# V-DETR/V-DETR

Hardware: AMD Instinct MI355X
Metric: scenes/sec (train fwd+bwd) 40k-pt ScanNet (higher is better)
Workload: dtype f32

## Files before the change

### include/vdetr_hip.h

```cpp
#ifndef VDETR_HIP_H
#define VDETR_HIP_H

#include <stddef.h>
#include <stdint.h>

#ifdef __cplusplus
extern "C" {
#endif

#define VDETR_OK 0
#define VDETR_ERR_ARG 1
#define VDETR_ERR_LAUNCH 2
#define VDETR_ERR_WORKSPACE 3

typedef void* vdetr_stream_t;

int vdetr_abi_version(void);
const char* vdetr_last_error(void);
int vdetr_ab_switches(void);


size_t vdetr_fps_workspace_bytes(int b, int n);
int vdetr_furthest_point_sampling_f32(const float* xyz, int b, int n, int m, int32_t* idx,
                                      void* workspace, size_t workspace_bytes, vdetr_stream_t stream);
// ... 327 lines not shown
  float *save_mean, *save_invstd;
  const float* pre_bias;
  int64_t* counters[8];
  int32_t ncounters;
  int32_t stats_given;
} vdetr_bnact_desc;

typedef struct vdetr_bnact_grads {
  const float* dy;
  float* dx;
  float *d_gamma, *d_beta;
  const float *sum_dy_xhat, *sum_dy, *inv_count;
} vdetr_bnact_grads;

int vdetr_relu_dropout_fwd_f32(const float* x, float* y, long n, float dropout_p, uint64_t seed, uint64_t offset,
                               const uint64_t* rng_state, vdetr_stream_t stream);
int vdetr_relu_dropout_bwd_f32(const float* y, const float* dy, float* dx, long n, float dropout_p, vdetr_stream_t stream);
int vdetr_bn_act_fwd_f32(const vdetr_bnact_desc* d, vdetr_stream_t stream);
int vdetr_bn_stats_f32(const vdetr_bnact_desc* d, float* mean, float* m2, vdetr_stream_t stream);
int vdetr_bn_act_bwd_f32(const vdetr_bnact_desc* d, const vdetr_bnact_grads* g, vdetr_stream_t stream);
int vdetr_bn_act_bwd_batch_f32(const vdetr_bnact_desc* descs, const vdetr_bnact_grads* grads, int n, vdetr_stream_t stream);

typedef struct vdetr_pack_entry {
  const void* src;
  uint64_t dst_offset;
  uint64_t numel;
} vdetr_pack_entry;
int vdetr_colsum_f32(const float* x, float* out, int rows, int cols, long row_stride, vdetr_stream_t stream);
size_t vdetr_colsum_workspace_bytes(int n, int rows, int cols);
int vdetr_colsum_batched_f32(const float* x, float* out, int n, int rows, int cols, long row_stride, long item_stride,
                             void* workspace, size_t workspace_bytes, vdetr_stream_t stream);
int vdetr_colsum_ptrs_f32(const float* const* items, float* out, int n, int rows, int cols, long row_stride, void* workspace,
                          size_t workspace_bytes, vdetr_stream_t stream);
int vdetr_pack_chunk_floats(void);
int vdetr_pack_f32(const vdetr_pack_entry* entries, const uint32_t* block_entry, const uint32_t* block_chunk, int nblocks,
                   float* dst, vdetr_stream_t stream);
int vdetr_pack_sumsq_f32(const vdetr_pack_entry* entries, const uint32_t* block_entry, const uint32_t* block_chunk, int nblocks,
                         float* dst, float* sumsq, vdetr_stream_t stream);

int vdetr_cpb_tables_f32(const float* coords, const float* w1, const float* b1, const float* w2, int n, int P, int hidden, int H,
                         float* hid_out, float* tables, vdetr_stream_t stream);

typedef struct vdetr_adamw_desc {
  float* param;
  const float* grad;
  float* exp_avg;
  float* exp_avg_sq;
  int64_t n;
  float* step;
  uint32_t* ticket;
  const float* sumsq;
  int32_t nsumsq;
  float max_norm;
  float norm_eps;
  float* norm_out;
  double lr, beta1, beta2, eps, weight_decay;
} vdetr_adamw_desc;
int vdetr_adamw_clip_f32(const vdetr_adamw_desc* d, vdetr_stream_t stream);
int vdetr_sumsq_blocks(long n);
int vdetr_sumsq_f32(const float* g, long n, float* partial, int npartial, vdetr_stream_t stream);

int vdetr_morton_sort_max(void);
int vdetr_morton_order_f32(const float* xyz, int B, int n, int* codes, long long* order, vdetr_stream_t stream);
int vdetr_topk_order_f32(const float* values, int B, int n, int nq, long long* order, vdetr_stream_t stream);

#define VDETR_GT_CORNERS 0
// ... 217 lines not shown
```

### v-detr_amd/_lib.py

```python
import ctypes
import os

import torch

_HERE = os.path.dirname(os.path.abspath(__file__))
LIB_PATH = os.path.join(_HERE, "lib", "libvdetr_hip.so")

c_int, c_float, c_void_p, c_size_t = ctypes.c_int, ctypes.c_float, ctypes.c_void_p, ctypes.c_size_t

VDETR_ATTN_SHARED_KV, VDETR_ATTN_PER_HEAD = 0, 1
VDETR_MASK_NONE, VDETR_MASK_BOOL, VDETR_MASK_FLOAT = 0, 1, 2


class AttnDesc(ctypes.Structure):

    _fields_ = [
        ("kind", ctypes.c_int32), ("B", ctypes.c_int32), ("H", ctypes.c_int32), ("nQ", ctypes.c_int32),
        ("nK", ctypes.c_int32), ("scale", c_float),
        ("table", c_void_p), ("table_size", ctypes.c_int32), ("log_scale", c_float), ("inv_log_norm", c_float),
        ("vertices", c_void_p), ("xyz", c_void_p), ("cos_sin", c_void_p),
        ("mask", c_void_p), ("mask_kind", ctypes.c_int32),
        ("dropout_p", c_float), ("seed", ctypes.c_uint64), ("offset", ctypes.c_uint64),
        ("rng_state", c_void_p),
        ("k_row_stride", ctypes.c_int32), ("v_row_stride", ctypes.c_int32),
# ... 182 lines not shown

class LsaProblem(ctypes.Structure):

    _fields_ = [(n, c_void_p) for n in ("cost_t", "nactual", "inds", "mask")] + [
        (n, ctypes.c_int32) for n in ("B", "P", "G", "row_repeat")]


class LsaBatch(ctypes.Structure):

    _fields_ = [("nproblems", ctypes.c_int32), ("reserved", ctypes.c_int32), ("p", LsaProblem * VDETR_LSA_MAX_PROBLEMS)]


_LOSS_W = ("w_cls", "w_angle_cls", "w_angle_reg", "w_center", "w_size", "w_giou")
_LOSS_PTR = ("cls_logits", "center_reg", "size_reg", "pre_center", "pre_size", "corners", "angle_logits", "angle_res_norm",
             "gt", "nactual", "inds", "mask", "labels", "num_boxes", "losses", "card_ws", "d_cls_logits", "d_center_reg", "d_size_reg",
             "d_corners", "d_angle_logits", "d_angle_res_norm", "rotated", "ce_rows_matched")


class SetLossDesc(ctypes.Structure):

    _fields_ = ([(n, ctypes.c_int32) for n in ("B", "P", "G", "C", "A", "label_override")] + [("focal_alpha", c_float)] +
                [(n, c_float) for n in _LOSS_W] + [("cls_kind", ctypes.c_int32), ("w_no_object", c_float)] +
                [(n, c_void_p) for n in _LOSS_PTR])


VDETR_IOU_GIOU, VDETR_IOU_DIOU, VDETR_IOU_IOU = 0, 1, 2
IOU_KINDS = {"giou": VDETR_IOU_GIOU, "diou": VDETR_IOU_DIOU, "iou": VDETR_IOU_IOU}


class IouExt(ctypes.Structure):

    _fields_ = [("iou_kind", ctypes.c_int32), ("reserved", ctypes.c_int32)] + [
        (n, c_void_p) for n in ("center", "size", "angle", "d_center", "d_size", "d_angle")]


class SpBnDesc(ctypes.Structure):

    _fields_ = ([(n, ctypes.c_int32) for n in ("N", "C", "act", "training")] + [("eps", c_float), ("momentum", c_float)] +
                [(n, c_void_p) for n in ("x", "gamma", "beta", "residual", "running_mean", "running_var", "num_batches_tracked",
                                         "y", "save_mean", "save_invstd", "workspace")])


_SIGNATURES = {
    "vdetr_abi_version": (c_int, []),
    "vdetr_ab_switches": (c_int, []),
    "vdetr_last_error": (ctypes.c_char_p, []),
    "vdetr_fps_workspace_bytes": (c_size_t, [c_int, c_int]),
    "vdetr_furthest_point_sampling_f32": (c_int, [c_void_p, c_int, c_int, c_int, c_void_p, c_void_p, c_size_t, c_void_p]),
    "vdetr_fps_varlen_workspace_bytes": (c_size_t, [c_void_p, c_int]),
    "vdetr_furthest_point_sampling_varlen_f32": (c_int, [c_void_p, c_void_p, c_int, c_int, c_void_p, c_void_p, c_size_t, c_void_p]),
    "vdetr_pos_embed_fourier_f32": (c_int, [c_void_p, c_int, c_int, c_void_p, c_void_p, c_void_p, c_int, c_int, c_void_p, c_void_p]),
    "vdetr_pos_embed_sine_f32": (c_int, [c_void_p, c_int, c_int, c_void_p, c_void_p, c_int, c_float, c_float, c_void_p, c_void_p]),
    "vdetr_gather_rows_f32": (c_int, [c_void_p, c_void_p, c_void_p, c_int, c_int, c_int, c_void_p]),
    "vdetr_gather_rows_grad_f32": (c_int, [c_void_p, c_void_p, c_void_p, c_int, c_int, c_int, c_void_p]),
    "vdetr_gather_points_f32": (c_int, [c_void_p, c_void_p, c_void_p, c_int, c_int, c_int, c_int, c_void_p]),
    "vdetr_gather_points_grad_f32": (c_int, [c_void_p, c_void_p, c_void_p, c_int, c_int, c_int, c_int, c_void_p]),
    "vdetr_gather_points_grad_set_f32": (c_int, [c_void_p, c_void_p, c_void_p, c_int, c_int, c_int, c_int, c_void_p]),
    "vdetr_group_points_grad_set_f32": (c_int, [c_void_p, c_void_p, c_void_p, c_int, c_int, c_int, c_int, c_int, c_void_p]),
    "vdetr_ball_query_f32": (c_int, [c_void_p, c_void_p, c_void_p, c_int, c_int, c_int, c_float, c_int, c_void_p]),
    "vdetr_group_points_f32": (c_int, [c_void_p, c_void_p, c_void_p, c_int, c_int, c_int, c_int, c_int, c_void_p]),
    "vdetr_group_points_grad_f32": (c_int, [c_void_p, c_void_p, c_void_p, c_int, c_int, c_int, c_int, c_int, c_void_p]),
    "vdetr_three_nn_f32": (c_int, [c_void_p, c_void_p, c_void_p, c_void_p, c_int, c_int, c_int, c_void_p]),
    "vdetr_three_interpolate_f32": (c_int, [c_void_p, c_void_p, c_void_p, c_void_p, c_int, c_int, c_int, c_int, c_void_p]),
    "vdetr_three_interpolate_grad_f32": (c_int, [c_void_p, c_void_p, c_void_p, c_void_p, c_int, c_int, c_int, c_int, c_void_p]),
    "vdetr_attn_fwd_workspace_bytes": (c_size_t, [ctypes.POINTER(AttnDesc)]),
    "vdetr_attn_kv_image_bytes": (c_size_t, [c_int, c_int]),
# ... 8 lines not shown
    "vdetr_attn_bwd_scores_f32": (c_int, [ctypes.POINTER(AttnDesc), c_void_p, c_void_p, c_void_p, c_void_p, c_void_p, c_void_p, c_void_p, c_void_p, c_size_t, c_void_p]),
    "vdetr_attn_bwd_kv_workspace_bytes": (c_size_t, [ctypes.POINTER(AttnDesc)]),
    "vdetr_attn_bwd_kv_f32": (c_int, [ctypes.POINTER(AttnDesc)] + [c_void_p] * 10 + [c_size_t, c_void_p]),
    "vdetr_attn_bwd_kv_delta_f32": (c_int, [ctypes.POINTER(AttnDesc)] + [c_void_p] * 11 + [c_size_t, c_void_p]),
    "vdetr_attn_bwd_dq_f32": (c_int, [ctypes.POINTER(AttnDesc), c_void_p, c_void_p, c_void_p, c_void_p]),
    "vdetr_attn_bwd_table_f32": (c_int, [ctypes.POINTER(AttnDesc), c_void_p, c_void_p, c_void_p, c_size_t, c_void_p]),
    "vdetr_attn_bwd_table_kernel_names": (c_int, [ctypes.POINTER(AttnDesc), ctypes.POINTER(ctypes.c_char_p), ctypes.POINTER(ctypes.c_char_p)]),
    "vdetr_attn_delta_f32": (c_int, [ctypes.POINTER(AttnDesc), c_void_p, c_void_p, c_void_p, c_void_p, c_void_p]),
    "vdetr_attn_dropout_mask_u8": (c_int, [ctypes.POINTER(AttnDesc), c_void_p, c_void_p]),
    "vdetr_rpe_bias_f32": (c_int, [ctypes.POINTER(AttnDesc), c_void_p, c_void_p]),
    "vdetr_box_decode_fwd_f32": (c_int, [ctypes.POINTER(BoxDecodeDesc), c_void_p]),
    "vdetr_box_decode_bwd_f32": (c_int, [ctypes.POINTER(BoxDecodeDesc), ctypes.POINTER(BoxDecodeGrads), c_void_p]),
    "vdetr_box_decode_bwd_batch_f32": (c_int, [ctypes.POINTER(BoxDecodeDesc), ctypes.POINTER(BoxDecodeGrads), c_int, c_void_p]),
    "vdetr_add_ln_fwd_f32": (c_int, [ctypes.POINTER(AddLnDesc), c_void_p]),
    "vdetr_add_ln_bwd_workspace_bytes": (c_size_t, [ctypes.POINTER(AddLnDesc)]),
    "vdetr_add_ln_bwd_f32": (c_int, [ctypes.POINTER(AddLnDesc), ctypes.POINTER(AddLnGrads), c_void_p]),
    "vdetr_add_ln_param_reduce_batch_f32": (c_int, [ctypes.POINTER(AddLnReduce), c_int, c_void_p]),
    "vdetr_relu_dropout_fwd_f32": (c_int, [c_void_p, c_void_p, ctypes.c_long, c_float, ctypes.c_uint64, ctypes.c_uint64, c_void_p,
                                           c_void_p]),
    "vdetr_relu_dropout_bwd_f32": (c_int, [c_void_p, c_void_p, c_void_p, ctypes.c_long, c_float, c_void_p]),
    "vdetr_bn_act_fwd_f32": (c_int, [ctypes.POINTER(BnActDesc), c_void_p]),
    "vdetr_bn_stats_f32": (c_int, [ctypes.POINTER(BnActDesc), c_void_p, c_void_p, c_void_p]),
    "vdetr_heads_workspace_bytes": (c_size_t, [c_int, c_int, c_int]),
    "vdetr_heads_fwd_f32": (c_int, [ctypes.POINTER(HeadsDesc), c_void_p]),
    "vdetr_pos_mlp_fwd_f32": (c_int, [ctypes.POINTER(PosMlpDesc), c_void_p]),
    "vdetr_heads_infer_f32": (c_int, [ctypes.POINTER(HeadsInferDesc), c_void_p]),
    "vdetr_pos_mlp_infer_f32": (c_int, [ctypes.POINTER(PosMlpDesc), c_void_p]),
    "vdetr_bn_act_bwd_f32": (c_int, [ctypes.POINTER(BnActDesc), ctypes.POINTER(BnActGrads), c_void_p]),
    "vdetr_bn_act_bwd_batch_f32": (c_int, [ctypes.POINTER(BnActDesc), ctypes.POINTER(BnActGrads), c_int, c_void_p]),
    "vdetr_colsum_f32": (c_int, [c_void_p, c_void_p, c_int, c_int, ctypes.c_long, c_void_p]),
    "vdetr_colsum_workspace_bytes": (c_size_t, [c_int, c_int, c_int]),
    "vdetr_colsum_batched_f32": (c_int, [c_void_p, c_void_p, c_int, c_int, c_int, ctypes.c_long, ctypes.c_long, c_void_p, c_size_t, c_void_p]),
    "vdetr_colsum_ptrs_f32": (c_int, [c_void_p, c_void_p, c_int, c_int, c_int, ctypes.c_long, c_void_p, c_size_t, c_void_p]),
    "vdetr_nms3d_workspace_bytes": (c_size_t, [c_int, c_int]),
    "vdetr_nms3d_f32": (c_int, [c_void_p, c_void_p, c_void_p, c_void_p, c_void_p, c_int, c_int, ctypes.c_double, c_int, c_void_p,
                        c_void_p, c_size_t, c_void_p]),
    "vdetr_nms3d_rot_workspace_bytes": (c_size_t, [c_int, c_int]),
    "vdetr_nms3d_rot_f32": (c_int, [c_void_p, c_void_p, c_void_p, c_void_p, c_void_p, c_int, c_int, ctypes.c_double, c_int, c_void_p,
                            c_void_p, c_size_t, c_void_p]),
    "vdetr_box_point_count_f32": (c_int, [c_void_p, c_void_p, c_int, c_int, c_int, c_void_p, c_void_p]),
    "vdetr_box3d_iou_max_f64": (c_int, [c_void_p, c_void_p, c_void_p, c_int, c_void_p, c_void_p, c_void_p, c_void_p, c_void_p,
                                c_void_p]),
    "vdetr_box3d_iou_pairs_f64": (c_int, [c_void_p, c_int, c_void_p, c_int, c_void_p, c_void_p]),
    "vdetr_morton_sort_max": (c_int, []),
    "vdetr_morton_order_f32": (c_int, [c_void_p, c_int, c_int, c_void_p, c_void_p, c_void_p]),
    "vdetr_pack_chunk_floats": (c_int, []),
    "vdetr_pack_f32": (c_int, [c_void_p, c_void_p, c_void_p, c_int, c_void_p, c_void_p]),
    "vdetr_pack_sumsq_f32": (c_int, [c_void_p, c_void_p, c_void_p, c_int, c_void_p, c_void_p, c_void_p]),
    "vdetr_adamw_clip_f32": (c_int, [ctypes.POINTER(AdamWDesc), c_void_p]),
    "vdetr_cpb_tables_f32": (c_int, [c_void_p] * 4 + [c_int] * 4 + [c_void_p] * 3),
    "vdetr_sumsq_blocks": (c_int, [ctypes.c_long]),
    "vdetr_sumsq_f32": (c_int, [c_void_p, ctypes.c_long, c_void_p, c_int, c_void_p]),
    "vdetr_gt_prepare_f32": (c_int, [c_void_p, c_int, c_int, c_int, c_void_p, c_void_p, c_void_p, c_void_p, c_void_p]),
    "vdetr_match_cost_f32": (c_int, [ctypes.POINTER(MatchDesc), c_void_p]),
    "vdetr_match_cost_batch_f32": (c_int, [ctypes.POINTER(MatchDesc), c_int, c_void_p]),
    "vdetr_lsa_f64": (c_int, [ctypes.POINTER(LsaBatch), c_void_p, c_void_p]),
    "vdetr_point_labels_f32": (c_int, [c_void_p, c_void_p, c_void_p, c_int, c_int, c_int, c_int, c_void_p, c_void_p, c_void_p]),
    "vdetr_set_loss_f32": (c_int, [ctypes.POINTER(SetLossDesc), c_void_p]),
    "vdetr_set_loss_batch_f32": (c_int, [ctypes.POINTER(SetLossDesc), c_int, c_void_p]),
    "vdetr_match_cost_ext_batch_f32": (c_int, [ctypes.POINTER(MatchDesc), ctypes.POINTER(IouExt), c_int, c_void_p]),
    "vdetr_set_loss_ext_batch_f32": (c_int, [ctypes.POINTER(SetLossDesc), ctypes.POINTER(IouExt), c_int, c_void_p]),
    "vdetr_sp_kernel_map_i32": (c_int, [c_void_p, c_int, c_void_p, c_int, c_void_p, c_int, c_void_p, c_void_p]),
    "vdetr_sp_inverse_map_i32": (c_int, [c_void_p, c_int, c_int, c_int, c_void_p, c_void_p]),
    "vdetr_sp_gather_cols_f32": (c_int, [c_void_p, c_void_p, c_int, c_int, c_int, c_void_p, c_void_p]),
    "vdetr_sp_gather_sum_f32": (c_int, [c_void_p, c_void_p, c_int, c_int, c_int, c_int, c_void_p, c_void_p]),
    "vdetr_sp_pairs_gemm_f32": (c_int, [c_void_p, c_void_p, c_void_p, c_void_p, c_int, c_int, c_int, c_int, c_void_p, c_void_p]),
# ... 60 lines not shown

def stream_ptr():
    return c_void_p(torch.cuda.current_stream().cuda_stream)


def ptr(t):
    return c_void_p(t.data_ptr()) if t is not None else c_void_p(0)


def require_gpu(t, name):
    if not t.is_cuda:
        raise RuntimeError(f"{name}: CPU not supported (tensor is on {t.device})")


def require_contiguous(t, name):
    if not t.is_contiguous():
        raise RuntimeError(f"{name} must be a contiguous tensor")


def require_float(t, name):
    if t.dtype != torch.float32:
        raise RuntimeError(f"{name} must be a float tensor")


def require_int(t, name):
    if t.dtype != torch.int32:
        raise RuntimeError(f"{name} must be an int tensor")


def workspace(nbytes, device):
    return torch.empty(max(int(nbytes), 1), dtype=torch.uint8, device=device)


_rocblas = {"lib": None, "handles": {}}
ROCBLAS_OP_N, ROCBLAS_OP_T = 111, 112


def rocblas():
    if _rocblas["lib"] is None:
        path = os.path.join(os.path.dirname(torch.__file__), "lib", "librocblas.so")
        rb = ctypes.CDLL(path if os.path.exists(path) else "librocblas.so")
        rb.rocblas_create_handle.argtypes = [ctypes.POINTER(c_void_p)]
        rb.rocblas_set_stream.argtypes = [c_void_p, c_void_p]
        rb.rocblas_sgemm_batched.argtypes = [c_void_p, c_int, c_int, c_int, c_int, c_int, c_void_p, c_void_p, c_int, c_void_p, c_int,
                                             c_void_p, c_void_p, c_int, c_int]
        _rocblas["lib"] = rb
    return _rocblas["lib"]


def sgemm_batched_ptrs(op_a, op_b, m, n, k, a_ptrs, lda, b_ptrs, ldb, c_ptrs, ldc, batch, device, alpha=1.0, beta=0.0):
    rb = rocblas()
    key = device.index if device.index is not None else torch.cuda.current_device()
    h = _rocblas["handles"].get(key)
    if h is None:
        if torch.cuda.is_current_stream_capturing():
            raise RuntimeError("rocBLAS handle: create it before a stream capture (run one step eagerly first)")
        h = c_void_p()
        with torch.cuda.device(key):
            if rb.rocblas_create_handle(ctypes.byref(h)) != 0:
                raise RuntimeError("rocblas_create_handle failed")
        _rocblas["handles"][key] = h
    if rb.rocblas_set_stream(h, c_void_p(torch.cuda.current_stream(device).cuda_stream)) != 0:
        raise RuntimeError("rocblas_set_stream failed")
    al, be = c_float(alpha), c_float(beta)
    addr = lambda p: c_void_p(p.data_ptr() if torch.is_tensor(p) else int(p))
    rc = rb.rocblas_sgemm_batched(h, op_a, op_b, m, n, k, ctypes.byref(al), addr(a_ptrs), lda, addr(b_ptrs), ldb, ctypes.byref(be),
                                  addr(c_ptrs), ldc, batch)
    if rc != 0:
        raise RuntimeError(f"rocblas_sgemm_batched failed (status {rc})")


_ptr_tables = {}


def upload_ptrs(ptrs, device):
    n = len(ptrs)
    key = device.index if device.index is not None else torch.cuda.current_device()
    T = _ptr_tables.get(key)
    if T is None:
        if torch.cuda.is_current_stream_capturing():
            raise RuntimeError("pointer tables: allocate before a stream capture (run one step eagerly first)")
        T = _ptr_tables[key] = {"ring": [torch.empty(1024, dtype=torch.int64).pin_memory() for _ in range(4)], "events": [None] * 4, "tick": 0,
                                "spare": [torch.empty(1024, dtype=torch.int64).pin_memory() for _ in range(48)], "kept": []}
    if n > 1024:
        raise RuntimeError(f"pointer table of {n} entries (max 1024)")
    dev = torch.empty(n, dtype=torch.int64, device=device)
    if torch.cuda.is_current_stream_capturing():
        if not T["spare"]:
            raise RuntimeError("pointer tables: more than 48 captured uploads in this process")
        host = T["spare"].pop()
        T["kept"].append(host)
        host[:n] = torch.tensor(ptrs, dtype=torch.int64)
        dev.copy_(host[:n], non_blocking=True)
        return dev
    slot = T["tick"] % 4
    T["tick"] += 1
    if T["events"][slot] is not None:
        T["events"][slot].synchronize()
    host = T["ring"][slot]
    host[:n] = torch.tensor(ptrs, dtype=torch.int64)
    dev.copy_(host[:n], non_blocking=True)
    ev = torch.cuda.Event()
    ev.record(torch.cuda.current_stream(device))
    T["events"][slot] = ev
    return dev
```

### v-detr_amd/helpers.py

```python
import copy
import os
from functools import partial

import torch
import torch.nn as nn


def colsum_batched(x3d):
    import ctypes
    from . import _lib as L
    assert x3d.dim() == 3 and x3d.stride(2) == 1
    n, rows, cols = x3d.shape
    lib = L.lib()
    need = lib.vdetr_colsum_workspace_bytes(n, rows, cols)
    ws = torch.empty(need, dtype=torch.uint8, device=x3d.device) if need else None
    out = torch.empty((n, cols), dtype=x3d.dtype, device=x3d.device)
    L.check(lib.vdetr_colsum_batched_f32(L.ptr(x3d), L.ptr(out), n, rows, cols, ctypes.c_long(x3d.stride(1)), ctypes.c_long(x3d.stride(0)),
                                         L.ptr(ws), need, L.stream_ptr()), "colsum_batched")
    return out


PTR_BATCH = os.environ.get("VDETR_PTR_BATCH", "1") != "0"


def _ptr_batchable(group):
    if not PTR_BATCH or len(group) > 256 or len(group) < 8:
        return False
    if torch.distributed.is_available() and torch.distributed.is_initialized() and torch.distributed.get_world_size() > 1:
        return False
    g0, x0 = group[0][2], group[0][3]
    if g0.shape[0] > 1024:
        return False
    if not (g0.is_cuda and g0.dtype == torch.float32 and x0.dtype == torch.float32 and g0.shape[1] % 4 == 0):
        return False
    for it in group:
        g, x = it[2], it[3]
        if not (g.stride(1) == 1 and x.stride(1) == 1 and g.stride(0) == g0.stride(0) and x.stride(0) == x0.stride(0)
                and g.stride(0) % 4 == 0 and g.data_ptr() % 16 == 0 and x.data_ptr() % 4 == 0):
            return False
    return True


def _wgrad_ptrs(group, need_w, need_b):
    import ctypes
    from . import _lib as L
    n = len(group)
    g0, x0 = group[0][2], group[0][3]
    rows, out_f, in_f = g0.shape[0], g0.shape[1], x0.shape[1]
    dev = g0.device
    dW = torch.empty((n, out_f, in_f), dtype=torch.float32, device=dev) if need_w else None
    dB = None
    ptrs = [it[3].data_ptr() for it in group] + [it[2].data_ptr() for it in group]
    if need_w:
        ptrs += [dW.data_ptr() + i * out_f * in_f * 4 for i in range(n)]
    tab = L.upload_ptrs(ptrs, dev)
    base = tab.data_ptr()
    if need_w:
        L.sgemm_batched_ptrs(L.ROCBLAS_OP_N, L.ROCBLAS_OP_T, in_f, out_f, rows, base, x0.stride(0), base + 8 * n, g0.stride(0),
                             base + 16 * n, in_f, n, dev)
    if need_b:
        lib = L.lib()
        dB = torch.empty((n, out_f), dtype=torch.float32, device=dev)
        need = lib.vdetr_colsum_workspace_bytes(n, rows, out_f)
        ws = torch.empty(need, dtype=torch.uint8, device=dev) if need else None
        L.check(lib.vdetr_colsum_ptrs_f32(ctypes.c_void_p(base + 8 * n), L.ptr(dB), n, rows, out_f, ctypes.c_long(g0.stride(0)), L.ptr(ws), need,
                                          L.stream_ptr()), "colsum_ptrs")
    if dW is not None:
        dW._ptr_table = tab
    elif dB is not None:
        dB._ptr_table = tab
    return dW, dB


def colsum(x2d):
    assert x2d.dim() == 2 and x2d.stride(1) == 1
    return colsum_batched(x2d.unsqueeze(0))[0]


class DeferredParamGrads:
    enabled = False
    pending = []

    @staticmethod
    def _view_of_leaf(p):
        if p is None or p.is_leaf or not p._is_view():
            return None
        base = p._base
        return base if base is not None and base.is_leaf and p.is_contiguous() and base.is_contiguous() else None

    @classmethod
    def _deliver(cls, p, g, roots, grads):
        if p.is_leaf and p.grad is None:
            p.grad = g
            return
        fn = p.grad_fn
        if type(fn).__name__ == "_AliasBackward":
            parts = _Alias.backward(fn, g)[2:]
            leaves = [nf[0].variable if nf[0] is not None and hasattr(nf[0], "variable") else None for nf in fn.next_functions]
            if len(leaves) == len(parts) and all(l is not None for l in leaves):
                for leaf, part in zip(leaves, parts):
                    cls._deliver(leaf, part, roots, grads)
                return
        roots.append(p)
        grads.append(g)

    @classmethod
    def leaves_of(cls, p):
        if p is None:
            return []
        if p.is_leaf:
            return [p]
        base = cls._view_of_leaf(p)
        if base is not None:
            return [base]
        fn = p.grad_fn
        if type(fn).__name__ == "_AliasBackward":
            leaves = [nf[0].variable if nf[0] is not None and hasattr(nf[0], "variable") else None for nf in fn.next_functions]
            if all(l is not None for l in leaves):
                return leaves
        return None

    @classmethod
    def flush(cls, select=None, collect=None, keepalive=None):
        if select is None:
            items, cls.pending = cls.pending, []
        else:
            items = [it for it in cls.pending if select(it)]
            cls.pending = [it for it in cls.pending if not select(it)]
        if not items:
            return
        if keepalive is not None:
            keepalive.extend(items)
        groups = {}
        for it in items:
            groups.setdefault((tuple(it[2].shape), tuple(it[3].shape)), []).append(it)
        roots, grads = [], []
        with torch.no_grad():
            for group in groups.values():
                n = len(group)
                if n == 1:
                    w, b, g2, x2 = group[0]
                    dW = torch.mm(g2.t(), x2)[None] if w is not None else None
                    dB = (colsum(g2 if g2.stride(1) == 1 else g2.contiguous()) if g2.is_cuda else g2.sum(0))[None] \
                        if b is not None else None
                else:
                    def order(e):
                        i, it = e
                        base = cls._view_of_leaf(it[0])
                        return (0, i, 0) if base is None else (1, id(base), it[0].storage_offset())
                    group = [it for _, it in sorted(enumerate(group), key=order)]
                    need_w, need_b = any(it[0] is not None for it in group), any(it[1] is not None for it in group)
                    if _ptr_batchable(group):
                        dW, dB = _wgrad_ptrs(group, need_w, need_b)
                    else:
                        G = torch.stack([it[2] for it in group])
                        dW = torch.bmm(G.transpose(1, 2), torch.stack([it[3] for it in group])) if need_w else None
                        dB = (colsum_batched(G) if G.is_cuda and G.dtype == torch.float32 else G.sum(1)) if need_b else None
                for which, R in ((0, dW), (1, dB)):
                    if R is None:
                        continue
                    i = 0
                    while i < n:
                        p = group[i][which]
                        if p is None:
                            i += 1
                            continue
                        base = cls._view_of_leaf(p)
                        k = 1
                        if base is not None and base.numel() % p.numel() == 0:
                            k = base.numel() // p.numel()
                            tiles = i + k <= n and all(
                                group[i + j][which] is not None and cls._view_of_leaf(group[i + j][which]) is base and
                                group[i + j][which].shape == p.shape and
                                group[i + j][which].storage_offset() == base.storage_offset() + j * p.numel() for j in range(k))
                            if tiles:
                                if collect is not None:
                                    collect.append((base, R[i:i + k].view(base.shape)))
                                else:
                                    cls._deliver(base, R[i:i + k].view(base.shape), roots, grads)
                                i += k
                                continue
                            k = 1
                        if collect is not None:
                            collect.append((p, R[i]))
                        else:
                            cls._deliver(p, R[i], roots, grads)
                        i += 1
        if roots:
            torch.autograd.backward(roots, grads)

# ... 388 lines not shown
```

### v-detr_amd/vdetr_transformer.py

```python
import copy
import itertools
import math
import os
from functools import partial
from typing import Optional

import numpy as np
import torch
import torch.nn.functional as F
from torch import Tensor, nn

from . import add_ln as ALN
from . import bn_act as BNA
from . import attention as A
from . import box_decode
from . import heads as HD
from . import rowblock as RB
from .helpers import (ACTIVATION_DICT, NORM_DICT, WEIGHT_INIT_DICT, GenericMLP, PointwiseConv1d,
                      PositionEmbeddingLearned, buffers_alias, cat_params, get_clones, linear, linear_pair, slot_stack_params,
                      stack_params)
from .pc_util import morton_argsort, scale_points, shift_scale_points

_salt_counter = itertools.count(1)

# ... 527 lines not shown

    @staticmethod
    def backward(ctx, *grads):
        recs, names = ctx.records, ctx.names
        S, K = len(recs), len(names)
        r0 = recs[0]
        Bsz, G, rows, N = r0["y"].shape
        C = r0["f"].shape[1]
        dev = r0["y"].device
        dY = torch.empty((S,) + tuple(r0["y"].shape), dtype=torch.float32, device=dev)
        box_decode.joint_backward_batch([(rec["meta"], rec["saved"], dict(zip(names, grads[s * K:(s + 1) * K])), dY[s])
                                         for s, rec in enumerate(recs)])
        one = Bsz == 1

        def fold(t, ch):
            t = t.reshape(S, Bsz, G, ch, N)
            return t.reshape(S * G, ch, N) if one else t.permute(0, 2, 3, 1, 4).reshape(S * G, ch, Bsz * N)

        def stack(k):
            st = [r["stack"] for r in recs]
            if k != "f" and all(x is not None and x[0] is st[0][0] and x[1] == i for i, x in enumerate(st)) and \
                    st[0][0][k].shape[0] == S:
                return st[0][0][k]
            return recs[0][k].unsqueeze(0) if S == 1 else torch.stack([r[k] for r in recs])

        h2, h1, f = stack("h2"), stack("h1"), stack("f")
        w3 = stack_params([r["w3"].detach().reshape(G, rows, C) for r in recs])
        w2 = stack_params([r["w2"].detach().reshape(G, C, C) for r in recs])
        w1 = stack_params([r["w1"].detach().reshape(G * C, C) for r in recs])
        from .helpers import DeferredParamGrads
        on_side = (dY.is_cuda and DeferredParamGrads.enabled and A.side_branch_in_use(dev) and not r0.get("inline_wg", False))

        def weight_grads(dx2, dx1):
            db3 = dY.sum(dim=(1, 4))
            dw3 = torch.bmm(fold(dY, rows), fold(h2, C).transpose(1, 2)).view(S, G, rows, C)
            dw2 = torch.bmm(fold(dx2, C), fold(h1, C).transpose(1, 2)).view(S, G, C, C)
            if one:
                dw1 = torch.bmm(dx1.view(S, G * C, N), f.view(S, C, N).transpose(1, 2))
            else:
                dw1 = torch.bmm(dx1.permute(0, 2, 1, 3).reshape(S, G * C, Bsz * N),
                                f.permute(0, 2, 1, 3).reshape(S, C, Bsz * N).transpose(1, 2))
            return db3, dw3, dw2, dw1

        dh2 = torch.matmul(w3.transpose(2, 3).unsqueeze(1), dY).view(S, Bsz, G * C, N)
        dx2 = torch.empty_like(dh2)
        dbn2 = BNA.backward_from_records([r["bn2"] for r in recs], [dh2[s] for s in range(S)], [dx2[s] for s in range(S)])
        dh1 = torch.matmul(w2.transpose(2, 3).unsqueeze(1), dx2.view(S, Bsz, G, C, N)).view(S, Bsz, G * C, N)
        dx1 = torch.empty_like(dh1)
        dbn1 = BNA.backward_from_records([r["bn1"] for r in recs], [dh1[s] for s in range(S)], [dx1[s] for s in range(S)])
        if one:
            dft = torch.bmm(dx1.view(S, G * C, N).transpose(1, 2), w1)
            out = [dft[s].view(N, 1, C) for s in range(S)]
        else:
            df = torch.matmul(w1.transpose(1, 2).unsqueeze(1), dx1)
            out = [df[s].permute(2, 0, 1) for s in range(S)]
        if on_side:
            def pairs_of(db3, dw3, dw2, dw1):
                pairs = []
                for s, r in enumerate(recs):
                    pairs += [(r["w1"], dw1[s].reshape(r["w1"].shape)), (r["w2"], dw2[s].reshape(r["w2"].shape)),
                              (r["w3"], dw3[s].reshape(r["w3"].shape)), (r["b3"], db3[s].reshape(r["b3"].shape))]
                return pairs
            for s in range(S):
                out += [None, dbn1[s][1], dbn1[s][2], None, dbn2[s][1], dbn2[s][2], None, None]
            A.side_late.append((lambda: pairs_of(*weight_grads(dx2, dx1)), (dY, h2, h1, f, dx2, dx1)))
            return (None, None, *out)
# ... 497 lines not shown
```

Before: 158.1.

## Add grouped split-K weight-gradient kernel using split-bf16 MFMA across parameter groups

Adds a HIP kernel that computes many weight-gradient GEMMs (plus bias column sums) in one launch. A device-side item table sets the tiling, and split-K partials go through a reduction kernel. Each fp32 operand is split into a bf16 high and low part and multiplied with three MFMA products, which approximates fp32 precision on matrix cores. It replaces the rocBLAS batched-pointer path and the separate colsum launch in the linear-layer grad batching and in the grouped conv MLP backward. The aim is to cut launch count and use matrix cores. The trade-off is lower precision than true fp32 and extra workspace traffic for the split-K partials.

```diff
diff --git a/include/vdetr_hip.h b/include/vdetr_hip.h
--- a/include/vdetr_hip.h
+++ b/include/vdetr_hip.h
@@ -383,6 +383,19 @@
                              void* workspace, size_t workspace_bytes, vdetr_stream_t stream);
 int vdetr_colsum_ptrs_f32(const float* const* items, float* out, int n, int rows, int cols, long row_stride, void* workspace,
                           size_t workspace_bytes, vdetr_stream_t stream);
+typedef struct vdetr_wgrad_item {
+  const float* a;
+  const float* b;
+  float* dw;
+  float* db;
+  int32_t M, N, K, flags;
+  int64_t a_sk, a_sm, b_sk, b_sn, ldw;
+  int32_t wg_begin, ksplit, kslice, tiles_n, red_begin, reserved;
+  int64_t ws_off;
+} vdetr_wgrad_item;
+int vdetr_wgrad_grouped_plan(vdetr_wgrad_item* items, int n, size_t* workspace_bytes);
+int vdetr_wgrad_grouped_f32(const vdetr_wgrad_item* host_items, const void* device_items, int n, void* workspace,
+                            size_t workspace_bytes, vdetr_stream_t stream);
 int vdetr_pack_chunk_floats(void);
 int vdetr_pack_f32(const vdetr_pack_entry* entries, const uint32_t* block_entry, const uint32_t* block_chunk, int nblocks,
                    float* dst, vdetr_stream_t stream);
diff --git a/v-detr_amd/_lib.py b/v-detr_amd/_lib.py
--- a/v-detr_amd/_lib.py
+++ b/v-detr_amd/_lib.py
@@ -238,6 +238,13 @@
 
     _fields_ = [("iou_kind", ctypes.c_int32), ("reserved", ctypes.c_int32)] + [
         (n, c_void_p) for n in ("center", "size", "angle", "d_center", "d_size", "d_angle")]
+
+
+class WgradItem(ctypes.Structure):
+
+    _fields_ = [(n, c_void_p) for n in ("a", "b", "dw", "db")] + [(n, ctypes.c_int32) for n in ("M", "N", "K", "flags")] + [
+        (n, ctypes.c_int64) for n in ("a_sk", "a_sm", "b_sk", "b_sn", "ldw")] + [
+        (n, ctypes.c_int32) for n in ("wg_begin", "ksplit", "kslice", "tiles_n", "red_begin", "reserved")] + [("ws_off", ctypes.c_int64)]
 
 
 class SpBnDesc(ctypes.Structure):
@@ -312,6 +319,8 @@
     "vdetr_colsum_workspace_bytes": (c_size_t, [c_int, c_int, c_int]),
     "vdetr_colsum_batched_f32": (c_int, [c_void_p, c_void_p, c_int, c_int, c_int, ctypes.c_long, ctypes.c_long, c_void_p, c_size_t, c_void_p]),
     "vdetr_colsum_ptrs_f32": (c_int, [c_void_p, c_void_p, c_int, c_int, c_int, ctypes.c_long, c_void_p, c_size_t, c_void_p]),
+    "vdetr_wgrad_grouped_plan": (c_int, [ctypes.POINTER(WgradItem), c_int, ctypes.POINTER(c_size_t)]),
+    "vdetr_wgrad_grouped_f32": (c_int, [ctypes.POINTER(WgradItem), c_void_p, c_int, c_void_p, c_size_t, c_void_p]),
     "vdetr_nms3d_workspace_bytes": (c_size_t, [c_int, c_int]),
     "vdetr_nms3d_f32": (c_int, [c_void_p, c_void_p, c_void_p, c_void_p, c_void_p, c_int, c_int, ctypes.c_double, c_int, c_void_p,
                         c_void_p, c_size_t, c_void_p]),
@@ -438,45 +447,8 @@
     return torch.empty(max(int(nbytes), 1), dtype=torch.uint8, device=device)
 
 
-_rocblas = {"lib": None, "handles": {}}
-ROCBLAS_OP_N, ROCBLAS_OP_T = 111, 112
-
-
-def rocblas():
-    if _rocblas["lib"] is None:
-        path = os.path.join(os.path.dirname(torch.__file__), "lib", "librocblas.so")
-        rb = ctypes.CDLL(path if os.path.exists(path) else "librocblas.so")
-        rb.rocblas_create_handle.argtypes = [ctypes.POINTER(c_void_p)]
-        rb.rocblas_set_stream.argtypes = [c_void_p, c_void_p]
-        rb.rocblas_sgemm_batched.argtypes = [c_void_p, c_int, c_int, c_int, c_int, c_int, c_void_p, c_void_p, c_int, c_void_p, c_int,
-                                             c_void_p, c_void_p, c_int, c_int]
-        _rocblas["lib"] = rb
-    return _rocblas["lib"]
-
-
-def sgemm_batched_ptrs(op_a, op_b, m, n, k, a_ptrs, lda, b_ptrs, ldb, c_ptrs, ldc, batch, device, alpha=1.0, beta=0.0):
-    rb = rocblas()
-    key = device.index if device.index is not None else torch.cuda.current_device()
-    h = _rocblas["handles"].get(key)
-    if h is None:
-        if torch.cuda.is_current_stream_capturing():
-            raise RuntimeError("rocBLAS handle: create it before a stream capture (run one step eagerly first)")
-        h = c_void_p()
-        with torch.cuda.device(key):
-            if rb.rocblas_create_handle(ctypes.byref(h)) != 0:
-                raise RuntimeError("rocblas_create_handle failed")
-        _rocblas["handles"][key] = h
-    if rb.rocblas_set_stream(h, c_void_p(torch.cuda.current_stream(device).cuda_stream)) != 0:
-        raise RuntimeError("rocblas_set_stream failed")
-    al, be = c_float(alpha), c_float(beta)
-    addr = lambda p: c_void_p(p.data_ptr() if torch.is_tensor(p) else int(p))
-    rc = rb.rocblas_sgemm_batched(h, op_a, op_b, m, n, k, ctypes.byref(al), addr(a_ptrs), lda, addr(b_ptrs), ldb, ctypes.byref(be),
-                                  addr(c_ptrs), ldc, batch)
-    if rc != 0:
-        raise RuntimeError(f"rocblas_sgemm_batched failed (status {rc})")
-
-
 _ptr_tables = {}
+PTR_TABLE_WORDS = 8192
 
 
 def upload_ptrs(ptrs, device):
@@ -486,17 +458,18 @@
     if T is None:
         if torch.cuda.is_current_stream_capturing():
             raise RuntimeError("pointer tables: allocate before a stream capture (run one step eagerly first)")
-        T = _ptr_tables[key] = {"ring": [torch.empty(1024, dtype=torch.int64).pin_memory() for _ in range(4)], "events": [None] * 4, "tick": 0,
-                                "spare": [torch.empty(1024, dtype=torch.int64).pin_memory() for _ in range(48)], "kept": []}
-    if n > 1024:
-        raise RuntimeError(f"pointer table of {n} entries (max 1024)")
+        T = _ptr_tables[key] = {"ring": [torch.empty(PTR_TABLE_WORDS, dtype=torch.int64).pin_memory() for _ in range(4)], "events": [None] * 4, "tick": 0,
+                                "spare": [torch.empty(PTR_TABLE_WORDS, dtype=torch.int64).pin_memory() for _ in range(48)], "kept": []}
+    if n > PTR_TABLE_WORDS:
+        raise RuntimeError(f"pointer table of {n} entries (max {PTR_TABLE_WORDS})")
+    words = ptrs if torch.is_tensor(ptrs) else torch.tensor(ptrs, dtype=torch.int64)
     dev = torch.empty(n, dtype=torch.int64, device=device)
     if torch.cuda.is_current_stream_capturing():
         if not T["spare"]:
             raise RuntimeError("pointer tables: more than 48 captured uploads in this process")
         host = T["spare"].pop()
         T["kept"].append(host)
-        host[:n] = torch.tensor(ptrs, dtype=torch.int64)
+        host[:n] = words
         dev.copy_(host[:n], non_blocking=True)
         return dev
     slot = T["tick"] % 4
@@ -504,7 +477,7 @@
     if T["events"][slot] is not None:
         T["events"][slot].synchronize()
     host = T["ring"][slot]
-    host[:n] = torch.tensor(ptrs, dtype=torch.int64)
+    host[:n] = words
     dev.copy_(host[:n], non_blocking=True)
     ev = torch.cuda.Event()
     ev.record(torch.cuda.current_stream(device))
diff --git a/v-detr_amd/csrc/wgrad_grouped.hip b/v-detr_amd/csrc/wgrad_grouped.hip
--- /dev/null
+++ b/v-detr_amd/csrc/wgrad_grouped.hip
@@ -0,0 +1,292 @@
+#include "common.h"
+
+namespace vdetr {
+
+typedef float wg_f32x4 __attribute__((ext_vector_type(4)));
+typedef float wg_f32x16 __attribute__((ext_vector_type(16)));
+typedef __bf16 wg_bf16x8 __attribute__((ext_vector_type(8)));
+typedef __bf16 wg_bf16x4 __attribute__((ext_vector_type(4)));
+
+constexpr int kWgTile = 128;
+constexpr int kWgStage = 32;
+constexpr int kWgRow = 40;
+constexpr int kWgReduceBlock = 1024;
+constexpr int kWgTargetWgs = 512;
+constexpr int kWgVecA = 1, kWgVecB = 2;
+
+__device__ __forceinline__ int wg_find(const vdetr_wgrad_item* items, int n, int bid, bool reduce) {
+  int lo = 0, hi = n - 1;
+  while (lo < hi) {
+    const int mid = (lo + hi + 1) >> 1;
+    const int begin = reduce ? items[mid].red_begin : items[mid].wg_begin;
+    if (begin <= bid) lo = mid; else hi = mid - 1;
+  }
+  return lo;
+}
+
+__device__ __forceinline__ void wg_load(const float* __restrict__ P, long sk, long sr, int r0, int R, int k, int k1, bool vec, int tid,
+                                        wg_f32x4 (&v)[4]) {
+  const int kg = tid & 7, q = tid >> 3;
+  if (sr == 1) {
+    const int c = r0 + 4 * q;
+#pragma unroll
+    for (int i = 0; i < 4; ++i) {
+      const int kk = k + 4 * kg + i;
+      v[i] = wg_f32x4{0.f, 0.f, 0.f, 0.f};
+      if (kk < k1 && c < R) {
+        const float* p = P + (long)kk * sk + c;
+        if (vec && c + 3 < R) {
+          v[i] = *reinterpret_cast<const wg_f32x4*>(p);
+        } else {
+#pragma unroll
+          for (int e = 0; e < 4; ++e)
+            if (c + e < R) v[i][e] = p[e];
+        }
+      }
+    }
+  } else {
+    const int kk = k + 4 * kg;
+#pragma unroll
+    for (int i = 0; i < 4; ++i) {
+      const int r = r0 + q + 32 * i;
+      v[i] = wg_f32x4{0.f, 0.f, 0.f, 0.f};
+      if (r < R && kk < k1) {
+        const float* p = P + (long)r * sr + kk;
+        if (vec && kk + 3 < k1) {
+          v[i] = *reinterpret_cast<const wg_f32x4*>(p);
+        } else {
+#pragma unroll
+          for (int e = 0; e < 4; ++e)
+            if (kk + e < k1) v[i][e] = p[e];
+        }
+      }
+    }
+  }
+}
+
+__device__ __forceinline__ void wg_put(__bf16* hi, __bf16* lo, int row, int kg, float x0, float x1, float x2, float x3) {
+  wg_bf16x4 h, l;
+  const float x[4] = {x0, x1, x2, x3};
+#pragma unroll
+  for (int e = 0; e < 4; ++e) {
+    const __bf16 t = (__bf16)x[e];
+    h[e] = t;
+    l[e] = (__bf16)(x[e] - (float)t);
+  }
+  *reinterpret_cast<wg_bf16x4*>(hi + row * kWgRow + 4 * kg) = h;
+  *reinterpret_cast<wg_bf16x4*>(lo + row * kWgRow + 4 * kg) = l;
+}
+
+__device__ __forceinline__ void wg_store(__bf16* hi, __bf16* lo, bool r_contig, int tid, const wg_f32x4 (&v)[4]) {
+  const int kg = tid & 7, q = tid >> 3;
+  if (r_contig) {
+#pragma unroll
+    for (int e = 0; e < 4; ++e) wg_put(hi, lo, 4 * q + e, kg, v[0][e], v[1][e], v[2][e], v[3][e]);
+  } else {
+#pragma unroll
+    for (int i = 0; i < 4; ++i) wg_put(hi, lo, q + 32 * i, kg, v[i][0], v[i][1], v[i][2], v[i][3]);
+  }
+}
+
+__global__ __launch_bounds__(256) void wgrad_grouped_kernel(const vdetr_wgrad_item* __restrict__ items, int nitems, float* __restrict__ ws) {
+  __shared__ __attribute__((aligned(16))) __bf16 img[2][2][kWgTile * kWgRow];
+  const int tid = threadIdx.x, lane = tid & 63, w = tid >> 6, wr = w >> 1, wc = w & 1, r31 = lane & 31, h = lane >> 5;
+  const vdetr_wgrad_item& it = items[wg_find(items, nitems, blockIdx.x, false)];
+  const int M = it.M, N = it.N, K = it.K, ksplit = it.ksplit, flags = it.flags;
+  const int local = blockIdx.x - it.wg_begin;
+  const int ks = local % ksplit, tile = local / ksplit, tn = tile % it.tiles_n, tm = tile / it.tiles_n;
+  const int m0 = tm * kWgTile, n0 = tn * kWgTile;
+  const int k0 = ks * it.kslice, k1 = k0 + it.kslice < K ? k0 + it.kslice : K;
+  const float* __restrict__ A = it.a;
+  const float* __restrict__ B = it.b;
+  const long a_sk = it.a_sk, a_sm = it.a_sm, b_sk = it.b_sk, b_sn = it.b_sn;
+  const bool a_rc = a_sm == 1, b_rc = b_sn == 1;
+  const bool want_db = it.db != nullptr && tn == 0;
+
+  wg_f32x16 acc[2][2];
+#pragma unroll
+  for (int i = 0; i < 2; ++i)
+#pragma unroll
+    for (int t = 0; t < 2; ++t)
+#pragma unroll
+      for (int e = 0; e < 16; ++e) acc[i][t][e] = 0.f;
+  float dbacc[4] = {0.f, 0.f, 0.f, 0.f};
+
+  wg_f32x4 va[4], vb[4];
+  if (k0 < k1) {
+    wg_load(A, a_sk, a_sm, m0, M, k0, k1, flags & kWgVecA, tid, va);
+    wg_load(B, b_sk, b_sn, n0, N, k0, k1, flags & kWgVecB, tid, vb);
+  }
+  for (int k = k0; k < k1; k += kWgStage) {
+    wg_store(img[0][0], img[0][1], a_rc, tid, va);
+    wg_store(img[1][0], img[1][1], b_rc, tid, vb);
+    if (want_db) {
+#pragma unroll
+      for (int e = 0; e < 4; ++e)
+        dbacc[e] += a_rc ? ((va[0][e] + va[1][e]) + (va[2][e] + va[3][e])) : ((va[e][0] + va[e][1]) + (va[e][2] + va[e][3]));
+    }
+    __syncthreads();
+    if (k + kWgStage < k1) {
+      wg_load(A, a_sk, a_sm, m0, M, k + kWgStage, k1, flags & kWgVecA, tid, va);
+      wg_load(B, b_sk, b_sn, n0, N, k + kWgStage, k1, flags & kWgVecB, tid, vb);
+    }
+#pragma unroll
+    for (int s = 0; s < 2; ++s) {
+      wg_bf16x8 ah[2], al[2], bh[2], bl[2];
+#pragma unroll
+      for (int i = 0; i < 2; ++i) {
+        const int off = (wr * 64 + 32 * i + r31) * kWgRow + 16 * s + 8 * h;
+        ah[i] = *reinterpret_cast<const wg_bf16x8*>(&img[0][0][off]);
+        al[i] = *reinterpret_cast<const wg_bf16x8*>(&img[0][1][off]);
+      }
+#pragma unroll
+      for (int t = 0; t < 2; ++t) {
+        const int off = (wc * 64 + 32 * t + r31) * kWgRow + 16 * s + 8 * h;
+        bh[t] = *reinterpret_cast<const wg_bf16x8*>(&img[1][0][off]);
+        bl[t] = *reinterpret_cast<const wg_bf16x8*>(&img[1][1][off]);
+      }
+#pragma unroll
+      for (int i = 0; i < 2; ++i)
+#pragma unroll
+        for (int t = 0; t < 2; ++t) {
+          acc[i][t] = __builtin_amdgcn_mfma_f32_32x32x16_bf16(al[i], bh[t], acc[i][t], 0, 0, 0);
+          acc[i][t] = __builtin_amdgcn_mfma_f32_32x32x16_bf16(ah[i], bl[t], acc[i][t], 0, 0, 0);
+          acc[i][t] = __builtin_amdgcn_mfma_f32_32x32x16_bf16(ah[i], bh[t], acc[i][t], 0, 0, 0);
+        }
+    }
+    __syncthreads();
+  }
+
+  const bool direct = ksplit == 1;
+  float* dst = direct ? it.dw : ws + it.ws_off + (size_t)ks * M * N;
+  const long ld = direct ? it.ldw : N;
+#pragma unroll
+  for (int i = 0; i < 2; ++i)
+#pragma unroll
+    for (int t = 0; t < 2; ++t) {
+      const int n = n0 + wc * 64 + 32 * t + r31;
+#pragma unroll
+      for (int e = 0; e < 16; ++e) {
+        const int m = m0 + wr * 64 + 32 * i + (e & 3) + 8 * (e >> 2) + 4 * h;
+        if (m < M && n < N) dst[(size_t)m * ld + n] = acc[i][t][e];
+      }
+    }
+  if (want_db) {
+    float* dbdst = direct ? it.db : ws + it.ws_off + (size_t)ksplit * M * N + (size_t)ks * M;
+    const int kg = tid & 7, q = tid >> 3;
+#pragma unroll
+    for (int e = 0; e < 4; ++e) {
+      float s = dbacc[e];
+      s += __shfl_xor(s, 1, 64);
+      s += __shfl_xor(s, 2, 64);
+      s += __shfl_xor(s, 4, 64);
+      const int m = m0 + (a_rc ? 4 * q + e : q + 32 * e);
+      if (kg == 0 && m < M) dbdst[m] = s;
+    }
+  }
+}
+
+__global__ __launch_bounds__(256) void wgrad_grouped_reduce_kernel(const vdetr_wgrad_item* __restrict__ items, int nitems,
+                                                                    const float* __restrict__ ws) {
+  const vdetr_wgrad_item& it = items[wg_find(items, nitems, blockIdx.x, true)];
+  const int M = it.M, N = it.N, ksplit = it.ksplit;
+  const long MN = (long)M * N, total = MN + (it.db ? M : 0);
+  const float* part = ws + it.ws_off;
+  const long base = (long)(blockIdx.x - it.red_begin) * kWgReduceBlock;
+#pragma unroll
+  for (int u = 0; u < kWgReduceBlock / 256; ++u) {
+    const long e = base + threadIdx.x + 256 * u;
+    if (e >= total) continue;
+    float s = 0.f;
+    if (e < MN) {
+      for (int c = 0; c < ksplit; ++c) s += part[(size_t)c * MN + e];
+      it.dw[(e / N) * it.ldw + e % N] = s;
+    } else {
+      const float* pb = part + (size_t)ksplit * MN + (e - MN);
+      for (int c = 0; c < ksplit; ++c) s += pb[(size_t)c * M];
+      it.db[e - MN] = s;
+    }
+  }
+}
+
+static int wg_plan(vdetr_wgrad_item* items, int n, bool fill, size_t* ws_bytes, int* wgs, int* red_blocks) {
+  VDETR_REQUIRE(items, "wgrad_grouped: null item table");
+  VDETR_REQUIRE(n >= 0 && n <= 4096, "wgrad_grouped: %d items (0 .. 4096)", n);
+  for (int i = 0; i < n; ++i) {
+    const vdetr_wgrad_item& it = items[i];
+    VDETR_REQUIRE(it.M >= 0 && it.N >= 0 && it.K >= 0, "wgrad_grouped: item %d: negative size (M=%d N=%d K=%d)", i, it.M, it.N, it.K);
+    VDETR_REQUIRE(it.M <= (1 << 20) && it.N <= (1 << 20) && it.K <= (1 << 24), "wgrad_grouped: item %d: size out of range", i);
+    if (it.M == 0 || it.N == 0) continue;
+    VDETR_REQUIRE(it.a && it.b && it.dw, "wgrad_grouped: item %d: null pointer", i);
+    VDETR_REQUIRE(((uintptr_t)it.a | (uintptr_t)it.b | (uintptr_t)it.dw | (uintptr_t)it.db) % 4 == 0,
+                  "wgrad_grouped: item %d: pointer not aligned to 4 bytes", i);
+    VDETR_REQUIRE((it.a_sk == 1 || it.a_sm == 1) && (it.b_sk == 1 || it.b_sn == 1) && it.a_sk >= 0 && it.a_sm >= 0 && it.b_sk >= 0 &&
+                      it.b_sn >= 0, "wgrad_grouped: item %d: each operand needs one unit stride and no negative one", i);
+    VDETR_REQUIRE(it.ldw >= it.N, "wgrad_grouped: item %d: dW row stride %ld < N = %d", i, (long)it.ldw, it.N);
+  }
+  auto tiles = [](const vdetr_wgrad_item& it) { return (long)ceil_div(it.M, kWgTile) * ceil_div(it.N, kWgTile); };
+  int L = 1024;
+  for (; L > 256; L /= 2) {
+    long total = 0;
+    for (int i = 0; i < n; ++i) total += tiles(items[i]) * (items[i].K > L ? ceil_div(items[i].K, L) : 1);
+    if (total >= kWgTargetWgs) break;
+  }
+  long wg = 0, red = 0, ws = 0;
+  for (int i = 0; i < n; ++i) {
+    vdetr_wgrad_item& it = items[i];
+    const int ksplit = it.K > L ? ceil_div(it.K, L) : 1;
+    const int kslice = ceil_div(ceil_div(it.K > 0 ? it.K : 1, ksplit), kWgStage) * kWgStage;
+    const int tiles_n = it.N > 0 ? ceil_div(it.N, kWgTile) : 1;
+    int flags = 0;
+    const long a_ld = it.a_sm == 1 ? it.a_sk : it.a_sm, b_ld = it.b_sn == 1 ? it.b_sk : it.b_sn;
+    if ((uintptr_t)it.a % 16 == 0 && a_ld % 4 == 0) flags |= kWgVecA;
+    if ((uintptr_t)it.b % 16 == 0 && b_ld % 4 == 0) flags |= kWgVecB;
+    if (fill) {
+      it.flags = flags; it.wg_begin = (int)wg; it.ksplit = ksplit; it.kslice = kslice; it.tiles_n = tiles_n; it.red_begin = (int)red;
+      it.reserved = 0; it.ws_off = ws;
+    } else {
+      VDETR_REQUIRE(it.flags == flags && it.wg_begin == (int)wg && it.ksplit == ksplit && it.kslice == kslice && it.tiles_n == tiles_n &&
+                        it.red_begin == (int)red && it.ws_off == ws,
+                    "wgrad_grouped: item %d does not carry the plan of vdetr_wgrad_grouped_plan (call it on the final table)", i);
+    }
+    wg += tiles(it) * ksplit;
+    if (ksplit > 1 && tiles(it) > 0) {
+      const long elems = (long)it.M * it.N + (it.db ? it.M : 0);
+      red += ceil_div(elems, kWgReduceBlock);
+      ws += (long)ksplit * elems;
+    }
+    VDETR_REQUIRE(wg < (1L << 30) && red < (1L << 30) && ws < (1L << 40), "wgrad_grouped: launch too large");
+  }
+  *ws_bytes = (size_t)ws * sizeof(float);
+  *wgs = (int)wg;
+  *red_blocks = (int)red;
+  return VDETR_OK;
+}
+
+}
+
+using namespace vdetr;
+
+extern "C" int vdetr_wgrad_grouped_plan(vdetr_wgrad_item* items, int n, size_t* workspace_bytes) {
+  VDETR_REQUIRE(workspace_bytes, "wgrad_grouped_plan: null pointer");
+  int wgs = 0, red = 0;
+  return wg_plan(items, n, true, workspace_bytes, &wgs, &red);
+}
+
+extern "C" int vdetr_wgrad_grouped_f32(const vdetr_wgrad_item* host_items, const void* device_items, int n, void* workspace,
+                                       size_t workspace_bytes, vdetr_stream_t stream) {
+  size_t need = 0;
+  int wgs = 0, red = 0;
+  const int rc = wg_plan(const_cast<vdetr_wgrad_item*>(host_items), n, false, &need, &wgs, &red);
+  if (rc != VDETR_OK) return rc;
+  if (wgs == 0) return VDETR_OK;
+  VDETR_REQUIRE(device_items && (uintptr_t)device_items % 8 == 0, "wgrad_grouped: device table null or not aligned to 8 bytes");
+  VDETR_REQUIRE(need == 0 || (workspace && workspace_bytes >= need && (uintptr_t)workspace % 16 == 0),
+                "wgrad_grouped: workspace of %zu bytes needed (got %zu)", need, workspace_bytes);
+  const vdetr_wgrad_item* dev = static_cast<const vdetr_wgrad_item*>(device_items);
+  hipLaunchKernelGGL(wgrad_grouped_kernel, dim3(wgs), dim3(256), 0, (hipStream_t)stream, dev, n, static_cast<float*>(workspace));
+  if (red > 0)
+    hipLaunchKernelGGL(wgrad_grouped_reduce_kernel, dim3(red), dim3(256), 0, (hipStream_t)stream, dev, n,
+                       static_cast<const float*>(workspace));
+  return check_launch("wgrad_grouped");
+}
diff --git a/v-detr_amd/helpers.py b/v-detr_amd/helpers.py
--- a/v-detr_amd/helpers.py
+++ b/v-detr_amd/helpers.py
@@ -23,53 +23,52 @@
 PTR_BATCH = os.environ.get("VDETR_PTR_BATCH", "1") != "0"
 
 
-def _ptr_batchable(group):
-    if not PTR_BATCH or len(group) > 256 or len(group) < 8:
+def _wg_operand_ok(t):
+    if not (t.is_cuda and t.dtype == torch.float32 and t.dim() in (2, 3)):
         return False
-    if torch.distributed.is_available() and torch.distributed.is_initialized() and torch.distributed.get_world_size() > 1:
-        return False
-    g0, x0 = group[0][2], group[0][3]
-    if g0.shape[0] > 1024:
-        return False
-    if not (g0.is_cuda and g0.dtype == torch.float32 and x0.dtype == torch.float32 and g0.shape[1] % 4 == 0):
-        return False
-    for it in group:
-        g, x = it[2], it[3]
-        if not (g.stride(1) == 1 and x.stride(1) == 1 and g.stride(0) == g0.stride(0) and x.stride(0) == x0.stride(0)
-                and g.stride(0) % 4 == 0 and g.data_ptr() % 16 == 0 and x.data_ptr() % 4 == 0):
-            return False
-    return True
-
-
-def _wgrad_ptrs(group, need_w, need_b):
+    k, r = t.shape[-2:]
+    sk, sr = t.stride()[-2:]
+    return (sk == 1 or sr == 1 or k == 1 or r == 1) and sk >= 0 and sr >= 0
+
+
+def wgrad_grouped(specs):
     import ctypes
     from . import _lib as L
-    n = len(group)
-    g0, x0 = group[0][2], group[0][3]
-    rows, out_f, in_f = g0.shape[0], g0.shape[1], x0.shape[1]
-    dev = g0.device
-    dW = torch.empty((n, out_f, in_f), dtype=torch.float32, device=dev) if need_w else None
-    dB = None
-    ptrs = [it[3].data_ptr() for it in group] + [it[2].data_ptr() for it in group]
-    if need_w:
-        ptrs += [dW.data_ptr() + i * out_f * in_f * 4 for i in range(n)]
-    tab = L.upload_ptrs(ptrs, dev)
-    base = tab.data_ptr()
-    if need_w:
-        L.sgemm_batched_ptrs(L.ROCBLAS_OP_N, L.ROCBLAS_OP_T, in_f, out_f, rows, base, x0.stride(0), base + 8 * n, g0.stride(0),
-                             base + 16 * n, in_f, n, dev)
-    if need_b:
-        lib = L.lib()
-        dB = torch.empty((n, out_f), dtype=torch.float32, device=dev)
-        need = lib.vdetr_colsum_workspace_bytes(n, rows, out_f)
-        ws = torch.empty(need, dtype=torch.uint8, device=dev) if need else None
-        L.check(lib.vdetr_colsum_ptrs_f32(ctypes.c_void_p(base + 8 * n), L.ptr(dB), n, rows, out_f, ctypes.c_long(g0.stride(0)), L.ptr(ws), need,
-                                          L.stream_ptr()), "colsum_ptrs")
-    if dW is not None:
-        dW._ptr_table = tab
-    elif dB is not None:
-        dB._ptr_table = tab
-    return dW, dB
+    flat = []
+    for A, B, dW, db in specs:
+        assert _wg_operand_ok(A) and _wg_operand_ok(B) and A.dim() == B.dim() == dW.dim() and A.shape[-2] == B.shape[-2]
+        assert tuple(dW.shape[-2:]) == (A.shape[-1], B.shape[-1]) and dW.dtype == torch.float32 and dW.is_cuda
+        assert (dW.stride(-1) == 1 or dW.shape[-1] == 1) and (db is None or (db.stride(-1) == 1 and db.dtype == torch.float32))
+        K, M, N = A.shape[-2], A.shape[-1], B.shape[-1]
+        a_sk, a_sm = (A.stride(-2), 1) if M == 1 else (1, A.stride(-1)) if K == 1 else A.stride()[-2:]
+        b_sk, b_sn = (B.stride(-2), 1) if N == 1 else (1, B.stride(-1)) if K == 1 else B.stride()[-2:]
+        ldw = max(dW.stride(-2), N)
+        nb = A.shape[0] if A.dim() == 3 else 1
+        assert A.dim() == 2 or (B.shape[0] == nb and dW.shape[0] == nb and (db is None or db.shape[0] == nb))
+        step = (lambda t: t.stride(0) * 4 if t.dim() == A.dim() and A.dim() == 3 else 0)
+        pa, pb, pw, pd = A.data_ptr(), B.data_ptr(), dW.data_ptr(), db.data_ptr() if db is not None else 0
+        sa, sb, sw, sd = step(A), step(B), step(dW), (db.stride(0) * 4 if db is not None and A.dim() == 3 else 0)
+        for i in range(nb):
+            flat.append((pa + i * sa, pb + i * sb, pw + i * sw, (pd + i * sd) or None, M, N, K, a_sk, a_sm, b_sk, b_sn, ldw))
+    n = len(flat)
+    if n == 0:
+        return None
+    arr = (L.WgradItem * n)()
+    for it, f in zip(arr, flat):
+        it.a, it.b, it.dw, it.db, it.M, it.N, it.K, it.a_sk, it.a_sm, it.b_sk, it.b_sn, it.ldw = f
+    dev = specs[0][0].device
+    lib = L.lib()
+    need = ctypes.c_size_t(0)
+    L.check(lib.vdetr_wgrad_grouped_plan(arr, n, ctypes.byref(need)), "wgrad_grouped_plan")
+    tab = L.upload_ptrs(torch.frombuffer(arr, dtype=torch.int64), dev)
+    ws = torch.empty(need.value, dtype=torch.uint8, device=dev) if need.value else None
+    with torch.cuda.device(dev):
+        L.check(lib.vdetr_wgrad_grouped_f32(arr, L.ptr(tab), n, L.ptr(ws), need.value, L.stream_ptr()), "wgrad_grouped")
+    return tab, ws
+
+
+def wgrad_grouped_usable(*tensors):
+    return PTR_BATCH and all(_wg_operand_ok(t) for t in tensors)
 
 
 def colsum(x2d):
@@ -136,26 +135,39 @@
             groups.setdefault((tuple(it[2].shape), tuple(it[3].shape)), []).append(it)
         roots, grads = [], []
         with torch.no_grad():
+            results, specs = [], []
             for group in groups.values():
                 n = len(group)
-                if n == 1:
-                    w, b, g2, x2 = group[0]
-                    dW = torch.mm(g2.t(), x2)[None] if w is not None else None
-                    dB = (colsum(g2 if g2.stride(1) == 1 else g2.contiguous()) if g2.is_cuda else g2.sum(0))[None] \
-                        if b is not None else None
-                else:
+                if n > 1:
                     def order(e):
                         i, it = e
                         base = cls._view_of_leaf(it[0])
                         return (0, i, 0) if base is None else (1, id(base), it[0].storage_offset())
                     group = [it for _, it in sorted(enumerate(group), key=order)]
-                    need_w, need_b = any(it[0] is not None for it in group), any(it[1] is not None for it in group)
-                    if _ptr_batchable(group):
-                        dW, dB = _wgrad_ptrs(group, need_w, need_b)
-                    else:
-                        G = torch.stack([it[2] for it in group])
-                        dW = torch.bmm(G.transpose(1, 2), torch.stack([it[3] for it in group])) if need_w else None
-                        dB = (colsum_batched(G) if G.is_cuda and G.dtype == torch.float32 else G.sum(1)) if need_b else None
+                need_w, need_b = any(it[0] is not None for it in group), any(it[1] is not None for it in group)
+                if need_w and all(wgrad_grouped_usable(it[2], it[3]) for it in group):
+                    g0, x0 = group[0][2], group[0][3]
+                    dW = torch.empty((n, g0.shape[1], x0.shape[1]), dtype=torch.float32, device=g0.device)
+                    dB = torch.empty((n, g0.shape[1]), dtype=torch.float32, device=g0.device) if need_b else None
+                    specs += [(it[2], it[3], dW[i], dB[i] if need_b else None, dW) for i, it in enumerate(group)]
+                elif n == 1:
+                    w, b, g2, x2 = group[0]
+                    dW = torch.mm(g2.t(), x2)[None] if w is not None else None
+                    dB = (colsum(g2 if g2.stride(1) == 1 else g2.contiguous()) if g2.is_cuda and g2.dtype == torch.float32
+                          else g2.sum(0))[None] if b is not None else None
+                else:
+                    G = torch.stack([it[2] for it in group])
+                    dW = torch.bmm(G.transpose(1, 2), torch.stack([it[3] for it in group])) if need_w else None
+                    dB = (colsum_batched(G) if G.is_cuda and G.dtype == torch.float32 else G.sum(1)) if need_b else None
+                results.append((group, dW, dB))
+            if specs:
+                by_dev = {}
+                for sp in specs:
+                    by_dev.setdefault(sp[0].device, []).append(sp)
+                for sub in by_dev.values():
+                    sub[0][4]._ptr_table = wgrad_grouped([sp[:4] for sp in sub])
+            for group, dW, dB in results:
+                n = len(group)
                 for which, R in ((0, dW), (1, dB)):
                     if R is None:
                         continue
diff --git a/v-detr_amd/vdetr_transformer.py b/v-detr_amd/vdetr_transformer.py
--- a/v-detr_amd/vdetr_transformer.py
+++ b/v-detr_amd/vdetr_transformer.py
@@ -583,6 +583,24 @@
         on_side = (dY.is_cuda and DeferredParamGrads.enabled and A.side_branch_in_use(dev) and not r0.get("inline_wg", False))
 
         def weight_grads(dx2, dx1):
+            from . import helpers as HP
+            wgrad_grouped = HP.wgrad_grouped
+            if HP.PTR_BATCH and DeferredParamGrads.enabled and all(t.is_cuda and t.dtype == torch.float32 for t in (dY, h2, h1, f, dx2, dx1)):
+                db3 = torch.empty((S, G, rows), dtype=torch.float32, device=dev)
+                dw3 = torch.empty((S, G, rows, C), dtype=torch.float32, device=dev)
+                dw2 = torch.empty((S, G, C, C), dtype=torch.float32, device=dev)
+                dw1 = torch.empty((S, G * C, C), dtype=torch.float32, device=dev)
+                kmaj = lambda t: t.transpose(1, 2)
+                if one:
+                    a1, b1 = dx1.view(S, G * C, N), f.view(S, C, N)
+                else:
+                    a1 = dx1.permute(0, 2, 1, 3).reshape(S, G * C, Bsz * N)
+                    b1 = f.permute(0, 2, 1, 3).reshape(S, C, Bsz * N)
+                dw3._ptr_table = wgrad_grouped([
+                    (kmaj(fold(dY, rows)), kmaj(fold(h2, C)), dw3.view(S * G, rows, C), db3.view(S * G, rows)),
+                    (kmaj(fold(dx2, C)), kmaj(fold(h1, C)), dw2.view(S * G, C, C), None),
+                    (kmaj(a1), kmaj(b1), dw1, None)])
+                return db3, dw3, dw2, dw1
             db3 = dY.sum(dim=(1, 4))
             dw3 = torch.bmm(fold(dY, rows), fold(h2, C).transpose(1, 2)).view(S, G, rows, C)
             dw2 = torch.bmm(fold(dx2, C), fold(h1, C).transpose(1, 2)).view(S, G, C, C)
```

After: 158.4, median of 2. No clear change (+0.2%).
